# TencentARC/SEED-Story

Hardware: AMD Instinct MI355X
Metric: story-steps/sec (text + 1024x1024 image) (higher is better)
Workload: dtype bf16

## Files before the change

### seed-story_amd/csrc/ss_gemm.hip

```cpp
#include <stdio.h>

#include <map>
#include <mutex>

#include "ss_gemm_common.h"

namespace ss {

__device__ __attribute__((aligned(16))) unsigned int g_zero_page[64];

template <typename T, int BM, int BN, int WM, int WN, int KT, bool CONV, bool SPLIT = false>
__global__ __launch_bounds__(64 * WM * WN) void gemm_kernel(const GemmArgs g) {
    static_assert(!SPLIT || Tr<T>::kVec == 4, "SPLIT: fp32 operands");
    constexpr int V = Tr<T>::kVec;
    constexpr int NT = 64 * WM * WN;
    constexpr int PPR = 8 * KT;
    constexpr int BK = PPR * V;
    constexpr int LS = BK + V;
    constexpr int TM = BM / WM, TN = BN / WN;
    constexpr int FM = TM / 16, FN = TN / 16;
    constexpr int PA = (BM * PPR + NT - 1) / NT, PW = (BN * PPR + NT - 1) / NT;
    static_assert(TM % 16 == 0 && TN % 16 == 0, "wave tile must be MFMA-shaped");

    extern __shared__ __attribute__((aligned(16))) char smem_raw[];
// ... 231 lines not shown
    }
    if (g.conv_Cin > 0)
        hipLaunchKernelGGL((gemm_kernel<T, BM, BN, WM, WN, KT, true>), grid, dim3(64 * WM * WN), lds, s, g);
    else
        hipLaunchKernelGGL((gemm_kernel<T, BM, BN, WM, WN, KT, false>), grid, dim3(64 * WM * WN), lds, s, g);
    SS_LAUNCH_CHECK("gemm");
    return SS_OK;
}

template <typename T, int BM, int BN, int WM, int WN, int NS, bool CONV>
__global__ __launch_bounds__(64 * WM * WN) void gemm_glds_kernel(const GemmArgs g) {
    constexpr int V = 8;
    constexpr int NW = WM * WN;
    constexpr int BK = 64;
    constexpr int TM = BM / WM, TN = BN / WN;
    constexpr int FM = TM / 16, FN = TN / 16;
    constexpr int IA = BM / 8 / NW, IW = BN / 8 / NW;
    static_assert(BM % (8 * NW) == 0 && BN % (8 * NW) == 0, "tile rows must split evenly over the waves");
    extern __shared__ __attribute__((aligned(16))) char smem_raw[];
    constexpr int TILE_BYTES = (BM + BN) * 128;

    const int tid = threadIdx.x, lane = tid & 63;
    const int wid = __builtin_amdgcn_readfirstlane(tid >> 6);
    const int wm = wid / WN, wn = wid % WN;
    const int l15 = lane & 15, grp = lane >> 4;
    int mt_, nt_;
    xcd_tile(g.swz, (g.M + BM - 1) / BM, (g.N + BN - 1) / BN, mt_, nt_);
    const int m_blk = mt_ * BM, n_blk = nt_ * BN;
    const T* __restrict__ A = (const T*)g.A;
    const T* __restrict__ W = (const T*)g.W;
    const int K = g.K, M = g.M, N = g.N;
    const int ntiles = (K + BK - 1) / BK;
    const T* zero = reinterpret_cast<const T*>(g_zero_page);
    const uint32_t lds0 = __builtin_amdgcn_readfirstlane((uint32_t)(size_t)(lds_void_t*)smem_raw);

    const int srow = lane >> 3;
    const int schunk = (lane & 7) ^ srow;
    int cb[IA], cy[IA], cx[IA];
    if constexpr (CONV) {
#pragma unroll
        for (int i = 0; i < IA; ++i) {
            const int m = m_blk + (wid * IA + i) * 8 + srow;
            const int hw = g.conv_Ho * g.conv_Wo;
            cb[i] = m / hw;
            const int rem = m - cb[i] * hw;
            cy[i] = rem / g.conv_Wo;
            cx[i] = rem - cy[i] * g.conv_Wo;
        }
    }
    auto issue_tile = [&](int t, int buf) {
        const int k = t * BK + schunk * V;
        const uint32_t base = lds0 + (uint32_t)(buf * TILE_BYTES);
#pragma unroll
        for (int i = 0; i < IA; ++i) {
            const int r8 = (wid * IA + i) * 8;
            const int m = m_blk + r8 + srow;
            const T* src = zero;
            if constexpr (CONV) {
                int tap, ci;
                if ((g.conv_Cin & 63) == 0) {
                    const int k0 = t * BK;
                    tap = k0 / g.conv_Cin;
                    ci = k0 - tap * g.conv_Cin + schunk * V;
                } else {
                    tap = k / g.conv_Cin;
                    ci = k - tap * g.conv_Cin;
                }
                const int dy = tap / 3 - 1, dx = tap - (tap / 3) * 3 - 1;
                int iy = cy[i] * g.conv_stride + dy, ix = cx[i] * g.conv_stride + dx;
                const int Hin = g.conv_up ? 2 * g.conv_H : g.conv_H, Win = g.conv_up ? 2 * g.conv_W : g.conv_W;
                const bool ok = m < M && k < K && iy >= 0 && iy < Hin && ix >= 0 && ix < Win;
                if (g.conv_up) { iy >>= 1; ix >>= 1; }
                if (ok) src = A + (((int64_t)cb[i] * g.conv_H + iy) * g.conv_W + ix) * g.conv_Cin + ci;
            } else {
                if (m < M && k < K) src = A + (int64_t)m * g.lda + k;
            }
            dma16(src, __builtin_amdgcn_readfirstlane(base + (uint32_t)(r8 * 128)));
        }
#pragma unroll
        for (int i = 0; i < IW; ++i) {
            const int r8 = (wid * IW + i) * 8;
            const int n = n_blk + r8 + srow;
            const T* src = (n < N && k < K) ? W + (int64_t)n * g.ldw + k : zero;
            dma16(src, __builtin_amdgcn_readfirstlane(base + (uint32_t)((BM + r8) * 128)));
        }
    };

    f32x4_t acc[FN][FM];
#pragma unroll
    for (int i = 0; i < FN; ++i)
#pragma unroll
        for (int j = 0; j < FM; ++j) acc[i][j] = f32x4_t{0.f, 0.f, 0.f, 0.f};

    constexpr int IPT = IA + IW;
#pragma unroll
    for (int st = 0; st < NS - 1; ++st)
        if (st < ntiles) issue_tile(st, st);
    int buf = 0;
    for (int t = 0; t < ntiles; ++t) {
        if (t + NS - 2 < ntiles) wait_vmcnt<(NS - 2) * IPT>();
        else wait_vmcnt<0>();
        __syncthreads();
        if (t + NS - 1 < ntiles) {
            int nb = buf + NS - 1;
            if (nb >= NS) nb -= NS;
            issue_tile(t + NS - 1, nb);
        }
        const char* abuf = smem_raw + buf * TILE_BYTES;
        if (++buf == NS) buf = 0;
        const char* wbuf = abuf + BM * 128;
#pragma unroll
        for (int ks = 0; ks < 2; ++ks) {
            uint4 fw[FN], fa[FM];
#pragma unroll
            for (int i = 0; i < FN; ++i) {
                const int r = wn * TN + i * 16 + l15;
                fw[i] = *reinterpret_cast<const uint4*>(wbuf + r * 128 + (((ks * 4 + grp) ^ (r & 7)) << 4));
            }
#pragma unroll
            for (int j = 0; j < FM; ++j) {
                const int r = wm * TM + j * 16 + l15;
                fa[j] = *reinterpret_cast<const uint4*>(abuf + r * 128 + (((ks * 4 + grp) ^ (r & 7)) << 4));
            }
#pragma unroll
            for (int i = 0; i < FN; ++i)
#pragma unroll
                for (int j = 0; j < FM; ++j) acc[i][j] = Mma<T>::run(fw[i], fa[j], acc[i][j]);
        }
    }

    gemm_epilogue<T, FM, FN>(g, acc, m_blk + wm * TM, n_blk + wn * TN, l15, grp);
}

template <typename T, int BM, int BN, int WM, int WN, int NS>
static int gemm_glds_launch_cfg(const GemmArgs& g, hipStream_t s) {
    if constexpr (Tr<T>::kVec == 8) {
        const size_t lds = (size_t)NS * (BM + BN) * 128;
        dim3 grid((unsigned)cdiv(g.N, BN), (unsigned)cdiv(g.M, BM));
        if (g.conv_Cin > 0)
            hipLaunchKernelGGL((gemm_glds_kernel<T, BM, BN, WM, WN, NS, true>), grid, dim3(64 * WM * WN), lds, s, g);
        else
            hipLaunchKernelGGL((gemm_glds_kernel<T, BM, BN, WM, WN, NS, false>), grid, dim3(64 * WM * WN), lds, s, g);
        SS_LAUNCH_CHECK("gemm_glds");
        return SS_OK;
    } else {
        return gemm_launch_cfg<T, 128, 128, 2, 2>(g, s);
    }
}

template <> int gemm_sp_dispatch<float>(int, const GemmArgs&, hipStream_t) { return 1; }
template <> int gemm_sp_dispatch_conv<float>(int, const GemmArgs&, hipStream_t) { return 1; }
template <> int gemm_pp_dispatch<float>(int, const GemmArgs&, hipStream_t) { return 1; }
template <> int gemm_pp_dispatch_conv<float>(int, const GemmArgs&, hipStream_t) { return 1; }
template <> int gemm_w4_dispatch<float>(int, const GemmArgs&, hipStream_t) { return 1; }
template <> int gemm_w4_dispatch_conv<float>(int, const GemmArgs&, hipStream_t) { return 1; }

template <typename T>
static int gemm_dispatch_cfg(int cfg, const GemmArgs& g, hipStream_t s) {
    if (cfg >= 90 && cfg < 100 && Tr<T>::kVec == 8) {
        const int rc = gemm_w4_run<T>(cfg, g, s);
        if (rc <= 0) return rc;
        cfg = g.conv_Cin > 0 ? 69 : 60;
    }
    if (cfg >= 50 && cfg < 60 && Tr<T>::kVec == 8) {
        const int rc = gemm_pp_run<T>(cfg, g, s);
        if (rc <= 0) return rc;
        cfg = g.conv_Cin > 0 ? 69 : 60;
    }
    if (cfg >= 20 && Tr<T>::kVec == 8) {
        const int rc = gemm_sp_run<T>(cfg, g, s);
        if (rc <= 0) return rc;
        const GemmTile t = sp_tile(cfg);
        cfg = t.BM == 64 ? 10 : (t.BM == 128 && t.BN == 64) ? 15 : 8;
    }
    switch (cfg) {
        case 1:
            if constexpr (Tr<T>::kVec == 4) {
                if (knob(K_gemm_f32_split)) {
                    const int st = knob(K_gemm_f32_split_tile);
                    if (st == 1 || (st == 0 && g.conv_Cin == 0 && g.M >= 2048 && g.N >= 8192)) return gemm_launch_cfg<T, 256, 128, 4, 2>(g, s);
                    if (st == 2) return gemm_launch_cfg<T, 128, 256, 2, 4>(g, s);
                }
            }
            return gemm_launch_cfg<T, 128, 128, 2, 2>(g, s);
        case 2: return gemm_launch_cfg<T, 64, 64, 2, 2>(g, s);
        case 8: return gemm_glds_launch_cfg<T, 128, 128, 2, 2, 2>(g, s);
        case 10: return gemm_glds_launch_cfg<T, 64, 64, 2, 2, 2>(g, s);
        case 15: return gemm_glds_launch_cfg<T, 128, 64, 2, 2, 2>(g, s);
        default:
            if (cfg >= 20) return gemm_launch_cfg<T, 128, 128, 2, 2>(g, s);
            return gemm_launch_cfg<T, 128, 32, 4, 1>(g, s);
    }
}

struct TuneKey {
    int32_t v[8];
    bool operator<(const TuneKey& o) const {
        for (int i = 0; i < 8; ++i) if (v[i] != o.v[i]) return v[i] < o.v[i];
        return false;
    }
};
static std::mutex g_tune_mutex;
static std::map<TuneKey, int>& tune_cache() {
    static std::map<TuneKey, int> m;
    return m;
}
static TuneKey make_key(int dtype, const GemmArgs& g) {
    const bool conv = g.conv_Cin > 0;
    const int Mk = conv ? g.M : (g.M + 127) / 128 * 128;
    return TuneKey{{dtype, Mk, g.N, g.K, g.conv_Cin, conv ? g.conv_stride * 2 + g.conv_up : 0, conv ? g.conv_H : 0,
                    conv ? g.conv_W : 0}};
}

static int pick_cfg(const GemmArgs& g, bool f32) {
    const int force = knob(K_gemm_cfg);
    if (force) return force;
    const int64_t M = g.M, N = g.N;
    if (M <= 128) return 3;
    if (f32) return 1;
    const bool sp_ok = (g.K % 64 == 0) && (g.conv_Cin == 0 || g.conv_Cin % 64 == 0);
    const int64_t t256 = (int64_t)cdiv(M, 256), t128 = (int64_t)cdiv(M, 128);
    if (sp_ok) {
        if (N % 160 == 0 && N < 2560) {
            if (t256 * (N / 160) >= 200) return 62;
            if (t128 * (N / 160) >= 200) return 61;
            return 67;
        }
        if (t256 * cdiv(N, 256) >= 200) return g.conv_Cin > 0 ? 69 : 60;
        if (N % 160 == 0 && t128 * (N / 160) >= 200) return 61;
        if (t128 * cdiv(N, 128) >= 256) return 65;
        return t128 * cdiv(N, 64) >= 256 ? 68 : 70;
    }
    return t128 * cdiv(N, 128) >= 256 ? 8 : 10;
}

template <typename T>
static int lookup_cfg(GemmArgs& g) {
    const int fallback = pick_cfg(g, Tr<T>::kVec != 8);
    if (Tr<T>::kVec != 8 || g.M <= 128 || knob(K_gemm_cfg) || !knob(K_gemm_table)) return fallback;
    const TuneKey key = make_key(Tr<T>::kDtype, g);
    std::lock_guard<std::mutex> lk(g_tune_mutex);
    auto it = tune_cache().find(key);
    if (it == tune_cache().end()) return fallback;
    g.swz = it->second / 100;
    return it->second % 100;
}

__global__ void tune_fill_kernel(uint16_t* p, size_t n, uint32_t seed, int is_bf16, float scale) {
    for (size_t i = (size_t)blockIdx.x * blockDim.x + threadIdx.x; i < n; i += (size_t)gridDim.x * blockDim.x) {
        uint32_t x = (uint32_t)i * 2654435761u + seed;
        x ^= x >> 15; x *= 2246822519u; x ^= x >> 13; x *= 3266489917u; x ^= x >> 16;
        const float f = ((float)(x >> 8) * (1.0f / 8388608.0f) - 1.0f) * scale;
        p[i] = is_bf16 ? (uint16_t)f32_to_bf16_bits(f) : (uint16_t)f32_to_f16_bits(f);
    }
}

static size_t tune_rot_bytes(size_t w_bytes) {
    const size_t wb = (w_bytes + 255) / 256 * 256;
    size_t n = ((size_t)352 << 20) / wb;
    if (n > 128) n = 128;
    if (n < 2) n = 2;
    return n * wb;
}

static const int kTuneCands[] = {8, 15, 10, 22, 54, 55, 56, 57, 58, 60, 61, 62, 63, 64, 65, 66, 67, 68, 69, 70, 71, 72};

template <typename T>
static int tune_shape(GemmArgs g, void* ws, size_t ws_bytes, size_t a_elems, hipStream_t s, float* best_us) {
    if constexpr (Tr<T>::kVec != 8) {
        return SS_OK;
    } else {
        const size_t e = sizeof(T);
        auto up = [](size_t b) { return (b + 255) / 256 * 256; };
        const size_t a_b = up(a_elems * e), w_b = up((size_t)g.N * g.K * e), c_b = up((size_t)g.M * g.N * e);
        SS_REQUIRE(ws && ws_bytes >= a_b + 2 * w_b + c_b, "tune: workspace too small (%zu bytes)", ws_bytes);
        int nW = (int)((ws_bytes - a_b - c_b) / w_b);
        if (nW > 128) nW = 128;
        char* p = (char*)ws;
        g.A = p; g.C = p + a_b;
        char* w0 = p + a_b + c_b;
        g.epi &= SS_EPI_GEGLU_PAIR | SS_EPI_GELU;
        if (g.epi & SS_EPI_GEGLU_PAIR) g.ldc = g.N / 2;
        hipLaunchKernelGGL(tune_fill_kernel, dim3(2048), dim3(256), 0, s, (uint16_t*)g.A, a_elems, 0x1234u,
                           Tr<T>::kDtype == SS_BF16, 1.0f);
        hipLaunchKernelGGL(tune_fill_kernel, dim3(2048), dim3(256), 0, s, (uint16_t*)w0, (size_t)nW * (w_b / e), 0x9876u,
                           Tr<T>::kDtype == SS_BF16, 0.05f);
        SS_LAUNCH_CHECK("tune_fill");
        hipEvent_t e0, e1;
        SS_HIP(hipEventCreate(&e0));
        SS_HIP(hipEventCreate(&e1));
        const int swzs[3] = {0, 4, 8};
        int best = -1, best_swz = 0;
        float best_ms = 1e30f;
        const bool log = knob(K_gemm_autotune_log) != 0;
        const int R = nW + nW / 2 > 12 ? nW + nW / 2 : 12;
        for (int c : kTuneCands) {
            for (int z : swzs) {
                g.swz = z;
                g.W = w0;
                if (c >= 50 && c < 60) {
                    const int rc = gemm_pp_run<T>(c, g, s);
                    if (rc != SS_OK) break;
                }
                if (gemm_dispatch_cfg<T>(c, g, s) != SS_OK) continue;
                g.W = w0 + w_b; gemm_dispatch_cfg<T>(c, g, s);
                hipEventRecord(e0, s);
// ... 496 lines not shown
```

### seed-story_amd/csrc/ss_gemm_common.h

```cpp
#pragma once
#include <type_traits>
#include <utility>

#include "ss_common.h"

namespace ss {

typedef __attribute__((ext_vector_type(4))) uint32_t u32x4_t;
typedef __attribute__((ext_vector_type(8))) uint32_t u32x8_t;
template <int NV> struct Frag { uint4 v[NV]; };
template <typename T> struct OutT { using type = T; };
template <> struct OutT<fp8_t> { using type = bf16_t; };
template <typename T> struct Mma;
template <> struct Mma<bf16_t> {
    static constexpr int kK = 32;
    static constexpr int kEB = 2;
    static constexpr int kNV = 1;
    static __device__ __forceinline__ f32x4_t run(const uint4& a, const uint4& b, f32x4_t c) {
        return __builtin_amdgcn_mfma_f32_16x16x32_bf16(__builtin_bit_cast(bf16x8_t, a),
                                                       __builtin_bit_cast(bf16x8_t, b), c, 0, 0, 0);
    }
    static __device__ __forceinline__ void run_inplace(const uint4& a, const uint4& b, f32x4_t& c) {
        asm volatile("v_mfma_f32_16x16x32_bf16 %0, %1, %2, %0"
                     : "+v"(c)
// ... 532 lines not shown
#pragma unroll
            for (int r = 0; r < 4; ++r) t[r] = acc[i][c][r] + bv[i][r];
            if constexpr (EV == 2) {
#pragma unroll
                for (int r = 0; r < 4; ++r) t[r] = gelu_for<T>(Tr<T>::rnd(t[r]));
            }
            if constexpr (EV == 3) {
                float rv[8];
                asm volatile("" : "+v"(rvp[i].x), "+v"(rvp[i].y));
                unpack<T>(make_uint4(rvp[i].x, rvp[i].y, 0u, 0u), rv);
#pragma unroll
                for (int r = 0; r < 4; ++r) t[r] = Tr<T>::rnd(t[r]) + rv[r];
            }
            if constexpr (GEGLU) {
                float v0, v1, v2, v3;
                unpack2<T>(pack2<T>(t[0], t[1]), v0, v1);
                unpack2<T>(pack2<T>(t[2], t[3]), v2, v3);
                const float o0 = v0 * Tr<T>::rnd(gelu_for<T>(v1)), o1 = v2 * Tr<T>::rnd(gelu_for<T>(v3));
                *reinterpret_cast<uint32_t*>(wrow + i * 16) = pack2<T>(o0, o1);
            } else {
                *reinterpret_cast<uint2*>(wrow + i * 32) = make_uint2(pack2<T>(t[0], t[1]), pack2<T>(t[2], t[3]));
            }
        }
    };
    uint4 u[NP];
    auto readback = [&]() {
#pragma unroll
        for (int k = 0; k < NP; ++k) u[k] = *reinterpret_cast<const uint4*>(stg + loff[k]);
    };

    constexpr int RD = 2;
    uint4 rr[FM][NP];
    auto row_ok = [&](int c, int k) { return pv[k] && (WHOLE || m_base + c * 16 + prow[k] < M); };
    auto load_res = [&](int c) {
        const gmem_char_t* Rc = uniform_gptr(Rb + c * rstep);
#pragma unroll
        for (int k = 0; k < NP; ++k) {
            if constexpr (WHOLE) rr[c][k] = gmem_ld16(Rc + roff[k]);
            else rr[c][k] = row_ok(c, k) ? gmem_ld16(Rc + roff[k]) : make_uint4(0u, 0u, 0u, 0u);
        }
    };
    load_rv(0);
    if (has_res) {
#pragma unroll
        for (int c = 0; c < RD && c < FM; ++c) load_res(c);
    }
    __builtin_amdgcn_sched_barrier(0);
    stage(0);
    __builtin_amdgcn_sched_barrier(0);
    readback();
#pragma unroll
    for (int c = 0; c < FM; ++c) {
        if (has_res && c + RD < FM) load_res(c + RD);
        __builtin_amdgcn_sched_barrier(0);
        if (c + 1 < FM) stage(c + 1);
        __builtin_amdgcn_sched_barrier(0);
        gmem_char_t* Cc = uniform_gptr(Cb + c * cstep);
#pragma unroll
        for (int k = 0; k < NP; ++k) {
            uint4 o = u[k];
            if (has_res) {
                float a[8], b[8];
                unpack<T>(o, a);
                unpack<T>(rr[c][k], b);
#pragma unroll
                for (int e = 0; e < 8; ++e) a[e] += b[e];
                o = pack<T>(a);
            }
            if (row_ok(c, k)) gmem_st16(Cc + goff[k], o);
        }
        __builtin_amdgcn_sched_barrier(0);
        if (c + 1 < FM) readback();
    }
}

#define SS_SP_TILES(X) \
    X(20, 128, 128, 2, 2, 1, 2,  0, 0) \
    X(21, 128,  64, 2, 2, 1, 2,  0, 0) \
    X(22,  64,  64, 2, 2, 1, 2,  0, 0) \
    X(23, 256, 128, 4, 2, 1, 2,  0, 0) \
    X(24, 256, 256, 2, 4, 2, 2,  0, 0)    \
    X(26, 128, 160, 2, 2, 1, 2,  0, 0)    \
    X(28, 128, 320, 2, 4, 1, 2,  0, 0)    \
    X(29,  64, 160, 2, 2, 1, 2,  0, 0)    \
    X(30, 256, 160, 4, 2, 1, 2,  0, 0)    \
    X(31, 256, 160, 4, 2, 1, 3,  0, 0)    \
    X(32, 256, 160, 4, 2, 1, 3,  1, 0)    \
    X(33, 256, 160, 4, 2, 1, 3,  3, 0)    \
    X(34, 256, 256, 2, 4, 2, 2,  1, 0)    \
    X(35, 256, 256, 2, 4, 2, 2,  2, 0)    \
    X(36, 256, 256, 2, 4, 2, 2,  3, 0)    \
    X(37, 128, 160, 2, 2, 1, 2,  1, 0)    \
    X(38, 256, 160, 4, 2, 1, 2,  2, 0)    \
    X(39, 128, 320, 2, 4, 1, 2,  2, 0)    \
    X(40, 256, 256, 2, 4, 2, 2,  6, 0)    \
    X(41, 128, 160, 2, 2, 1, 2,  4, 0)    \
    X(42, 256, 160, 4, 2, 1, 3,  4, 0)    \
    X(43, 256, 160, 4, 2, 1, 2,  6, 0)    \
    X(44, 128, 320, 2, 4, 1, 2,  4, 0)    \
    X(45, 256, 128, 4, 2, 1, 2,  4, 0)    \
    X(46, 128, 128, 2, 2, 1, 2,  4, 0)    \
    X(60, 256, 256, 2, 4, 2, 2, 11, 1)    \
    X(61, 128, 160, 2, 2, 1, 2,  8, 3)    \
    X(62, 256, 160, 4, 2, 1, 3, 12, 3)    \
    X(63, 128, 320, 2, 4, 1, 2,  8, 3)    \
    X(64, 256, 160, 4, 2, 1, 2, 10, 3)    \
    X(65, 128, 128, 2, 2, 1, 2,  8, 3)    \
    X(66, 256, 128, 4, 2, 1, 2,  8, 1)    \
    X(67,  64, 160, 2, 2, 1, 2,  8, 3)    \
    X(68, 128,  64, 2, 2, 1, 2,  8, 1)    \
    X(69, 256, 256, 2, 4, 2, 2,  8, 1)    \
    X(70,  64,  64, 2, 2, 1, 2,  8, 1)    \
    X(71, 256, 160, 4, 2, 1, 2,  8, 3)    \
    X(72, 128, 320, 2, 4, 1, 2, 10, 3)
#define SS_SP_SPLITK_TILES(X) \
    X(300, 128, 128, 2, 2, 1, 2, 64, 0) \
    X(301, 128,  64, 2, 2, 1, 2, 64, 0)
#define SS_SP_FP8_TILES(X) \
    X(80, 128, 128, 2, 2, 2, 2, 8, 0)     \
    X(81, 128, 160, 2, 2, 2, 2, 8, 0)     \
    X(82, 256, 160, 4, 2, 2, 2, 8, 0)     \
    X(85,  64, 160, 2, 2, 1, 2, 8, 0)     \
    X(86,  64,  64, 2, 2, 1, 2, 8, 0) \
    X(88, 128, 160, 2, 2, 2, 2, 0, 0)
#define SS_W4_FP8_TILES(X) \
    X(95, 256, 256, 2, 2, 16, 0, 2, 0)    \
    X(96, 256, 256, 2, 2, 16, 0, 0, 0)

struct GemmTile { int id, BM, BN, WM, WN, NH, NS, FLAGS, variants; };
#define SS_TILE_ROW(id, BM, BN, WM, WN, NH, NS, FLAGS, VAR) {id, BM, BN, WM, WN, NH, NS, FLAGS, VAR},
constexpr GemmTile kSpTiles[] = {SS_SP_TILES(SS_TILE_ROW)};
constexpr GemmTile kFp8Tiles[] = {SS_SP_FP8_TILES(SS_TILE_ROW) SS_W4_FP8_TILES(SS_TILE_ROW)};
template <int N> constexpr GemmTile find_tile(const GemmTile (&t)[N], int id) {
    for (int i = 0; i < N; ++i) if (t[i].id == id) return t[i];
    return GemmTile{};
}
constexpr GemmTile sp_tile(int id) { return find_tile(kSpTiles, id); }
constexpr GemmTile fp8_tile(int id) { return find_tile(kFp8Tiles, id); }

template <int N> constexpr bool tiles_well_formed(const GemmTile (&t)[N]) {
    for (int i = 0; i < N; ++i) {
        for (int j = 0; j < i; ++j) if (t[j].id == t[i].id) return false;
        if (t[i].id < 1 || t[i].id >= 100 || (t[i].variants && !(t[i].FLAGS & 8))) return false;
    }
    return true;
}
static_assert(tiles_well_formed(kSpTiles) && tiles_well_formed(kFp8Tiles),
              "tile lists: duplicate id, base id outside 1 .. 99, or a variant on a tile without the staged epilogue");

template <typename T> int gemm_sp_dispatch(int cfg, const GemmArgs& g, hipStream_t s);
template <typename T> int gemm_sp_dispatch_conv(int cfg, const GemmArgs& g, hipStream_t s);
template <typename T> int gemm_pp_dispatch(int cfg, const GemmArgs& g, hipStream_t s);
template <typename T> int gemm_pp_dispatch_conv(int cfg, const GemmArgs& g, hipStream_t s);
template <typename T> int gemm_w4_dispatch(int cfg, const GemmArgs& g, hipStream_t s);
template <typename T> int gemm_w4_dispatch_conv(int cfg, const GemmArgs& g, hipStream_t s);
int gemm_sp_dispatch_fp8(int cfg, const GemmArgs& g, hipStream_t s);
int gemm_w4_dispatch_fp8(int cfg, const GemmArgs& g, hipStream_t s);
template <typename T> static int gemm_sp_run(int cfg, const GemmArgs& g, hipStream_t s) {
    return g.conv_Cin > 0 ? gemm_sp_dispatch_conv<T>(cfg, g, s) : gemm_sp_dispatch<T>(cfg, g, s);
}
template <typename T> static int gemm_pp_run(int cfg, const GemmArgs& g, hipStream_t s) {
    return g.conv_Cin > 0 ? gemm_pp_dispatch_conv<T>(cfg, g, s) : gemm_pp_dispatch<T>(cfg, g, s);
}
template <typename T> static int gemm_w4_run(int cfg, const GemmArgs& g, hipStream_t s) {
    return g.conv_Cin > 0 ? gemm_w4_dispatch_conv<T>(cfg, g, s) : gemm_w4_dispatch<T>(cfg, g, s);
}

static inline int num_cus() {
    static int n = 0;
    if (!n) {
        int dev = 0;
        hipDeviceProp_t p;
        if (hipGetDevice(&dev) == hipSuccess && hipGetDeviceProperties(&p, dev) == hipSuccess) n = p.multiProcessorCount;
        if (n <= 0) n = 256;
    }
    return n;
}
template <auto KERN> static int launch_tiles(const char* name, const GemmArgs& g, int total, int cap, int threads, size_t lds, hipStream_t s) {
    const int grid = cap > 0 && total > cap ? cap : total;
    if (lds > 64 * 1024) SS_DYN_LDS(KERN, lds);
    hipLaunchKernelGGL(KERN, dim3((unsigned)grid, (unsigned)g.ksplit), dim3(threads), lds, s, g, total);
    SS_LAUNCH_CHECK(name);
    return SS_OK;
}

}
```

### seed-story_amd/csrc/ss_gemm_pp.inc

```

namespace ss {

template <int BN, int FLAGS>
struct PpLds {
    static constexpr int FN = BN / 64, FN0 = (FN + 1) / 2, FN1 = FN / 2, TN = FN * 16;
    static constexpr int HA = 128 * 128, HB0 = 4 * FN0 * 16 * 128, HB1 = 4 * FN1 * 16 * 128;
    static constexpr int BUF = 2 * HA + HB0 + HB1;
    static constexpr int STG_CR = 16, STG_WAVE = STG_CR * (TN * 2 + 16);
    static constexpr bool STG_IN_RING = 2 * BUF + 8 * STG_WAVE > 163840;
    static constexpr int BYTES = 2 * BUF + ((FLAGS & 8) != 0 && !STG_IN_RING ? 8 * STG_WAVE : 0);
};

static __device__ __attribute__((aligned(4096))) unsigned int g_pp_zero_page[1024];

__device__ __forceinline__ void dma16v(const char* gsrc, uint32_t lds_base) {
    asm volatile(
        "s_mov_b32 m0, %1\n\t"
        "s_nop 0\n\t"
        "global_load_lds_dwordx4 %0, off"
        :
        : "v"(gsrc), "s"(lds_base)
        : "memory");
}

__device__ __forceinline__ void dma16s_at(uint32_t voff, const void* sbase, uint32_t lds_wave, int off) {
    asm volatile(
        "s_add_u32 m0, %2, %3\n\t"
        "s_nop 0\n\t"
        "global_load_lds_dwordx4 %0, %1"
        :
        : "v"(voff), "s"(sbase), "s"(lds_wave), "i"(off)
        : "memory", "scc");
}
__device__ __forceinline__ void dma16v_at(const char* gsrc, uint32_t lds_wave, int off) {
    asm volatile(
        "s_add_u32 m0, %1, %2\n\t"
        "s_nop 0\n\t"
        "global_load_lds_dwordx4 %0, off"
        :
        : "v"(gsrc), "s"(lds_wave), "i"(off)
        : "memory", "scc");
}

__device__ __forceinline__ uint32_t sel_lanes(uint32_t a, uint32_t b, uint64_t mask) {
    uint32_t r;
    asm("v_cndmask_b32 %0, %1, %2, %3" : "=v"(r) : "v"(a), "v"(b), "s"(mask));
    return r;
}
__device__ __forceinline__ uint64_t uniform_u64(uint64_t v) {
    const uint32_t lo = __builtin_amdgcn_readfirstlane((uint32_t)v), hi = __builtin_amdgcn_readfirstlane((uint32_t)(v >> 32));
    return ((uint64_t)hi << 32) | lo;
}

template <typename T, int BN, int FLAGS, bool CONV>
__global__ __launch_bounds__(512) void gemm_pp_kernel(const GemmArgs g, const int total_tiles) {
    using Lds = PpLds<BN, FLAGS>;
    constexpr int BM = 256, FN = Lds::FN, FN0 = Lds::FN0, FN1 = Lds::FN1, TM = 128, TN = Lds::TN, FM = 8;
    static_assert(BN == 256 || BN == 320, "tile widths");
    constexpr bool EXACT = BN == 320 || CONV;
    constexpr bool PRIO = (FLAGS & 1) != 0, PERSIST = (FLAGS & 2) != 0, TWO = (FLAGS & 4) != 0, STAGED = (FLAGS & 8) != 0, RSTAT = (FLAGS & 32) != 0;
    constexpr int EM = ((FLAGS & 16) != 0) ? 2 : 0;
    constexpr int HA = Lds::HA, HB0 = Lds::HB0, HB1 = Lds::HB1, BUF = Lds::BUF;
    constexpr int OFF_A0 = 0, OFF_A1 = HA, OFF_B0 = 2 * HA, OFF_B1 = 2 * HA + HB0;
    constexpr int NP0 = FN0, NP1 = FN1;
    constexpr int FLY = NP0 + 2 + NP1;
    constexpr int STG_CR = Lds::STG_CR, STG_WAVE = Lds::STG_WAVE;
    constexpr bool STG_IN_RING = Lds::STG_IN_RING;
    static_assert(!(PERSIST && STG_IN_RING), "persistent tiles prefetch under the epilogue: the strips need their own LDS");
    static_assert(Mma<T>::kEB == 2, "16-bit operands");
    using TO = T;
    extern __shared__ __attribute__((aligned(16))) char smem_raw[];

    const int tid = threadIdx.x, lane = tid & 63;
    const int wid = __builtin_amdgcn_readfirstlane(tid >> 6);
    const int wm = wid >> 2, wn = wid & 3;
    const int l15 = lane & 15, grp = lane >> 4;
    const int M = g.M, N = g.N;
    const int MT = (M + BM - 1) / BM, NT = (N + BN - 1) / BN;
    const int ntiles = g.K / 64;
    const int tpt = CONV ? g.conv_Cin / 64 : 1;
    const uint32_t tpt_inv = CONV ? (65536u + (uint32_t)tpt - 1u) / (uint32_t)tpt : 0u;
    const int lw = CONV ? __builtin_ctz((unsigned)g.conv_W) : 0;
    const uint32_t lds0 = __builtin_amdgcn_readfirstlane((uint32_t)(size_t)(lds_void_t*)smem_raw);

    const int srow = lane >> 3;
    const int schunk = (lane & 7) ^ srow;
    auto b_col = [&](int h, int i) {
        const int RH = (h ? FN1 : FN0) * 16;
        const int r8 = (wid + 8 * i) * 8;
        return (r8 / RH) * TN + (h ? FN0 * 16 : 0) + r8 % RH + srow;
    };
    int m_blk = 0, n_blk = 0;
    uint32_t voffA[EXACT ? 1 : 2][EXACT ? 1 : 2], voffW[EXACT ? 1 : 2][EXACT ? 1 : 3];
    const char* sbaseA = nullptr;
    const char* sbaseW = nullptr;
    uint32_t cpoff[CONV ? 2 : 1][CONV ? 2 : 1];
    uint64_t cpad = 0, crow = 0;
    auto setup_tile = [&](int vid) {
        int mt_, nt_;
        xcd_tile_id(g.swz, MT, NT, vid, mt_, nt_);
        m_blk = mt_ * BM; n_blk = nt_ * BN;
        if constexpr (CONV) {
            voffA[0][0] = (uint32_t)(srow * g.conv_Cin * 2 + schunk * 16);
            voffW[0][0] = (uint32_t)((int64_t)srow * g.ldw * 2 + schunk * 16);
            uint64_t pad = 0, row = 0;
#pragma unroll
            for (int h = 0; h < 2; ++h) {
#pragma unroll
                for (int i = 0; i < 2; ++i) {
                    const int m0 = m_blk + i * 128 + h * 64 + wid * 8;
                    const int y0 = (m0 >> lw) & (g.conv_H - 1), x0 = m0 & (g.conv_W - 1);
                    const uint64_t r9 = (y0 == 0 ? 0x000000111ull : 0ull) | (y0 == g.conv_H - 1 ? 0x111000000ull : 0ull);
                    const uint64_t p9 = r9 | (x0 == 0 ? 0x001001001ull : 0ull) | (x0 + 8 == g.conv_W ? 0x100100100ull : 0ull);
                    row |= r9 << (h * 2 + i);
                    pad |= p9 << (h * 2 + i);
                    cpoff[h][i] = __builtin_amdgcn_readfirstlane((uint32_t)(m0 * g.conv_Cin * 2));
                }
            }
            cpad = uniform_u64(pad); crow = uniform_u64(row);
        } else if constexpr (EXACT) {
            voffA[0][0] = (uint32_t)((int64_t)srow * g.lda * 2 + schunk * 16);
            voffW[0][0] = (uint32_t)((int64_t)srow * g.ldw * 2 + schunk * 16);
        } else {
#pragma unroll
            for (int h = 0; h < 2; ++h) {
#pragma unroll
                for (int i = 0; i < 2; ++i) {
                    int m = m_blk + i * 128 + h * 64 + wid * 8 + srow;
                    m = m < M ? m : M - 1;
                    voffA[h][i] = (uint32_t)((int64_t)(m - m_blk) * g.lda * 2 + schunk * 16);
                }
#pragma unroll
                for (int i = 0; i < (h ? NP1 : NP0); ++i) {
                    int n = n_blk + b_col(h, i);
                    n = n < N ? n : N - 1;
                    voffW[h][i] = (uint32_t)((int64_t)(n - n_blk) * g.ldw * 2 + schunk * 16);
                }
            }
        }
        sbaseA = uniform_ptr((const char*)g.A + (CONV ? (int64_t)0 : (int64_t)m_blk * g.lda * 2));
        sbaseW = uniform_ptr((const char*)g.W + (int64_t)n_blk * g.ldw * 2);
    };
    struct Cur { const char* src; int c, tap; uint32_t bits; };
    auto cur_set_tap = [&](Cur& k) {
        const int t3 = (k.tap * 11) >> 5;
        const int dy = t3 - 1, dx = k.tap - 3 * t3 - 1;
        k.src = (const char*)g.A + ((int64_t)(dy * g.conv_W + dx) * g.conv_Cin + k.c * 64) * 2;
        k.bits = ((uint32_t)(cpad >> (k.tap * 4)) & 15u) | (((uint32_t)(crow >> (k.tap * 4)) & 15u) << 4) | (dx < 0 ? 256u : 0u);
    };
    auto cur_make = [&](int t) {
        Cur k;
        k.tap = (int)(((uint32_t)t * tpt_inv) >> 16);
        k.c = t - k.tap * tpt;
        cur_set_tap(k);
        return k;
    };
    auto cur_next = [&](Cur& k) {
        k.c += 1; k.src += 128;
        if (k.c == tpt) { k.c = 0; k.tap += 1; cur_set_tap(k); }
    };
    const uint32_t ldsw = lds0 + (uint32_t)(wid * 1024);
    const uint64_t zaddr = (uint64_t)(size_t)g_pp_zero_page;
    const uint32_t zlo = (uint32_t)zaddr | (uint32_t)((tid & 255) << 4);
    uint32_t zhi = (uint32_t)(zaddr >> 32);
    if constexpr (CONV && BN == 256) asm volatile("" : "+v"(zhi));
    auto stage_conv = [&](const Cur& k, int b, int h) {
        const uint32_t keep = m0_save();
#pragma unroll
        for (int i = 0; i < 2; ++i) {
            const int p = h * 2 + i;
            const char* ps = k.src + cpoff[CONV ? h : 0][CONV ? i : 0];
            const int d = b * BUF + (h ? OFF_A1 : OFF_A0) + i * 8192;
            if (__builtin_expect(((k.bits >> p) & 1u) == 0, 1)) {
                dma16s_at(voffA[0][0], ps, ldsw, d);
            } else {
                const uint64_t zm = ((k.bits >> (4 + p)) & 1u) ? ~0ull : ((k.bits & 256u) ? 0xFFull : 0xFFull << 56);
                const uint64_t a = (uint64_t)(size_t)ps + voffA[0][0];
                const uint32_t lo = sel_lanes((uint32_t)a, zlo, zm), hi = sel_lanes((uint32_t)(a >> 32), zhi, zm);
                dma16v_at((const char*)(size_t)(((uint64_t)hi << 32) | lo), ldsw, d);
            }
        }
        m0_restore(keep);
    };
    auto stage = [&](int t, int b, int which) {
        const uint32_t keep = m0_save();
        const int h = which & 1;
        if (which < 2) {
            const uint32_t dst = lds0 + (uint32_t)(b * BUF + (h ? OFF_A1 : OFF_A0) + wid * 1024);
            const char* src = sbaseA + (int64_t)t * 128;
#pragma unroll
            for (int i = 0; i < 2; ++i) {
                if constexpr (CONV) {
                } else if constexpr (EXACT)
                    dma16s(voffA[0][0], uniform_ptr(src + (int64_t)(i * 128 + h * 64 + wid * 8) * g.lda * 2), __builtin_amdgcn_readfirstlane(dst + i * 8192u));
                else
                    dma16s(voffA[h][i], src, __builtin_amdgcn_readfirstlane(dst + i * 8192u));
            }
        } else {
            const uint32_t dst = lds0 + (uint32_t)(b * BUF + (h ? OFF_B1 : OFF_B0) + wid * 1024);
            const char* src = sbaseW + (int64_t)t * 128;
#pragma unroll
            for (int i = 0; i < (h ? NP1 : NP0); ++i) {
                if constexpr (CONV)
                    dma16s_at(voffW[0][0], src + (uint32_t)__builtin_amdgcn_readfirstlane((b_col(h, i) - srow) * g.ldw * 2), ldsw,
                              b * BUF + (h ? OFF_B1 : OFF_B0) + i * 8192);
                else if constexpr (EXACT)
                    dma16s(voffW[0][0], uniform_ptr(src + (int64_t)(b_col(h, i) - srow) * g.ldw * 2), __builtin_amdgcn_readfirstlane(dst + i * 8192u));
                else
                    dma16s(voffW[h][i], src, __builtin_amdgcn_readfirstlane(dst + i * 8192u));
            }
        }
        m0_restore(keep);
    };
    auto prologue = [&]() {
        if constexpr (CONV) {
            const Cur k0 = cur_make(0);
            stage(0, 0, 2); stage_conv(k0, 0, 0); stage(0, 0, 3); stage_conv(k0, 0, 1);
            if (ntiles > 1) { stage_conv(cur_make(1), 1, 0); stage(1, 1, 2); if constexpr (!TWO) stage(1, 1, 3); }
        } else {
            stage(0, 0, 2); stage(0, 0, 0); stage(0, 0, 3); stage(0, 0, 1);
            if (ntiles > 1) { stage(1, 1, 0); stage(1, 1, 2); if constexpr (!TWO) stage(1, 1, 3); }
        }
    };

    const uint32_t fsw = (uint32_t)((grp ^ (l15 & 7)) << 4);
    const uint32_t fa0 = (uint32_t)((wm * 64 + l15) * 128) + fsw, fa1 = fa0 ^ 64u;
    const uint32_t fw00 = (uint32_t)((wn * FN0 * 16 + l15) * 128) + fsw, fw01 = fw00 ^ 64u;
    const uint32_t fw10 = (uint32_t)((wn * FN1 * 16 + l15) * 128) + fsw, fw11 = fw10 ^ 64u;
    uint4 fa[4][2], fw0[FN0][2], fw1[FN1][2];
    auto read_a = [&](const char* half) {
#pragma unroll
        for (int j = 0; j < 4; ++j) {
            fa[j][0] = *reinterpret_cast<const uint4*>(half + fa0 + j * 2048);
            fa[j][1] = *reinterpret_cast<const uint4*>(half + fa1 + j * 2048);
        }
    };
    auto read_w0 = [&](const char* half) {
#pragma unroll
        for (int i = 0; i < FN0; ++i) {
            fw0[i][0] = *reinterpret_cast<const uint4*>(half + fw00 + i * 2048);
            fw0[i][1] = *reinterpret_cast<const uint4*>(half + fw01 + i * 2048);
        }
    };
    auto read_w1 = [&](const char* half) {
#pragma unroll
        for (int i = 0; i < FN1; ++i) {
            fw1[i][0] = *reinterpret_cast<const uint4*>(half + fw10 + i * 2048);
            fw1[i][1] = *reinterpret_cast<const uint4*>(half + fw11 + i * 2048);
        }
    };
    f32x4_t acc[FN][FM];
    auto mma = [&](int h, auto hp_tag) {
        constexpr int hp = decltype(hp_tag)::value;
        if constexpr (PRIO) __builtin_amdgcn_s_setprio(1);
#pragma unroll
        for (int ks = 0; ks < 2; ++ks)
#pragma unroll
            for (int i = 0; i < (hp ? FN1 : FN0); ++i)
#pragma unroll
                for (int j = 0; j < 4; ++j) {
                    if constexpr (hp == 0) Mma<T>::run_inplace(fw0[i][ks], fa[j][ks], acc[i][h * 4 + j]);
                    else Mma<T>::run_inplace(fw1[i][ks], fa[j][ks], acc[FN0 + i][h * 4 + j]);
                }
        if constexpr (PRIO) __builtin_amdgcn_s_setprio(0);
    };
    constexpr std::integral_constant<int, 0> H0{};
    constexpr std::integral_constant<int, 1> H1{};
    auto bar = [&]() { __builtin_amdgcn_s_barrier(); };
    auto pin = [&]() { __builtin_amdgcn_sched_barrier(0); };

    int vid = blockIdx.x;
    setup_tile(vid);
    prologue();
    bool first = true;

    while (true) {
        const int m_cur = m_blk, n_cur = n_blk;
        const int vnext = vid + (int)gridDim.x;
        const bool has_next = PERSIST && vnext < total_tiles;
#pragma unroll
        for (int i = 0; i < FN; ++i)
#pragma unroll
            for (int j = 0; j < FM; ++j) acc[i][j] = f32x4_t{0.f, 0.f, 0.f, 0.f};
        if (first && ntiles > 1) wait_vmcnt<(TWO ? 2 + NP0 : FLY)>(); else wait_vmcnt<0>();
        first = false;
        bar();
#pragma unroll
        for (int i = 0; i < FN; ++i)
#pragma unroll
            for (int j = 0; j < FM; ++j) asm volatile("" : "+v"(acc[i][j]));
        asm volatile("s_nop 7" ::: "memory");
        if (wm == 1) bar();
        Cur P1 = cur_make(CONV ? 1 : 0), P2 = cur_make(CONV ? 2 : 0);

        auto tile = [&](int t, auto btag) {
            constexpr int b = decltype(btag)::value;
            const char* L = smem_raw + b * BUF;
            const bool s1 = t + 1 < ntiles, s2 = t + 2 < ntiles;
            read_w0(L + OFF_B0);
            pin();
            read_a(L + OFF_A0);
            pin();
            if (s1) { if constexpr (CONV) stage_conv(P1, b ^ 1, 1); else stage(t + 1, b ^ 1, 1); }
            asm volatile("s_waitcnt lgkmcnt(8)" ::: "memory");
            bar();
            asm volatile("s_waitcnt lgkmcnt(0)" ::: "memory");
            pin();
            mma(0, H0);
            pin();
            bar();
            read_w1(L + OFF_B1);
            pin();
            if (s2) stage(t + 2, b, 2);
            bar();
            asm volatile("s_waitcnt lgkmcnt(0)" ::: "memory");
            pin();
            mma(0, H1);
            pin();
            bar();
            read_a(L + OFF_A1);
            pin();
            if (s2) { if constexpr (CONV) stage_conv(P2, b, 0); else stage(t + 2, b, 0); }
            bar();
            asm volatile("s_waitcnt lgkmcnt(0)" ::: "memory");
            pin();
            mma(1, H1);
            pin();
            bar();
            if (s2) { stage(t + 2, b, 3); wait_vmcnt<FLY>(); } else { wait_vmcnt<0>(); }
            bar();
            pin();
            mma(1, H0);
            pin();
            bar();
            if constexpr (CONV) { P1 = P2; cur_next(P2); }
        };
        auto tile2 = [&](int t, auto btag) {
            constexpr int b = decltype(btag)::value;
            const char* L = smem_raw + b * BUF;
            const bool s1 = t + 1 < ntiles, s2 = t + 2 < ntiles;
            read_w0(L + OFF_B0);
            read_w1(L + OFF_B1);
            read_a(L + OFF_A0);
            pin();
            if (s1) {
                stage(t + 1, b ^ 1, 3);
                if constexpr (CONV) stage_conv(P1, b ^ 1, 1); else stage(t + 1, b ^ 1, 1);
                wait_vmcnt<4 + NP0 + NP1>();
            } else {
                wait_vmcnt<0>();
            }
            asm volatile("s_waitcnt lgkmcnt(0)" ::: "memory");
            bar();
            pin();
            mma(0, H0);
            mma(0, H1);
            pin();
            bar();
            read_a(L + OFF_A1);
            pin();
            if (s2) {
                if constexpr (CONV) stage_conv(P2, b, 0); else stage(t + 2, b, 0);
                stage(t + 2, b, 2);
                wait_vmcnt<4 + NP0>();
            } else if (s1) {
                wait_vmcnt<2>();
            } else {
                wait_vmcnt<0>();
            }
            asm volatile("s_waitcnt lgkmcnt(0)" ::: "memory");
            bar();
            pin();
            mma(1, H1);
            mma(1, H0);
            pin();
            bar();
            if constexpr (CONV) { P1 = P2; cur_next(P2); }
        };
        int t = 0;
        for (; t + 1 < ntiles; t += 2) {
            if constexpr (TWO) { tile2(t, std::integral_constant<int, 0>{}); tile2(t + 1, std::integral_constant<int, 1>{}); }
            else { tile(t, std::integral_constant<int, 0>{}); tile(t + 1, std::integral_constant<int, 1>{}); }
        }
        if (t < ntiles) { if constexpr (TWO) tile2(t, std::integral_constant<int, 0>{}); else tile(t, std::integral_constant<int, 0>{}); }
        if (wm == 0) bar();

        if (has_next) {
            setup_tile(vnext);
            prologue();
        }
        asm volatile("s_nop 15\n\ts_nop 15" ::: "memory");
#pragma unroll
        for (int i = 0; i < FN; ++i)
#pragma unroll
            for (int j = 0; j < FM; ++j) asm volatile("" : "+v"(acc[i][j]));

        bool staged = false;
        if constexpr (STAGED) {
            constexpr size_t A16 = 15;
            staged = (n_cur + wn * TN + TN <= N) && (((size_t)g.C | (size_t)g.residual | (size_t)g.bias | (size_t)g.rowvec) & A16) == 0 &&
                     ((g.ldc | g.ldr | g.rowvec_ld) & 7) == 0 && (EM == 0 || ((size_t)g.scale_w & A16) == 0);
            if (staged) {
                char* strip = smem_raw + (STG_IN_RING ? 0 : 2 * BUF) + wid * STG_WAVE;
                const int mb = m_cur + wm * TM, nb = n_cur + wn * TN;
                const bool o_gelu = (g.epi & SS_EPI_GELU) != 0, o_geglu = (g.epi & SS_EPI_GEGLU_PAIR) != 0;
                const bool o_rv = g.rowvec != nullptr || (!CONV && (g.epi & SS_EPI_INTERNAL_GENERIC) != 0);
                if constexpr (EM == 0 && !RSTAT) {
                    const bool o_res = (g.epi & SS_EPI_RESIDUAL) != 0;
                    if (!o_gelu && !o_geglu && !o_rv && !o_res) gemm_epilogue_staged_pipe<TO, FM, FN, 1, false, EXACT>(g, acc, mb, nb, lane, strip);
                    else if (!o_gelu && !o_geglu && !o_rv) gemm_epilogue_staged_pipe<TO, FM, FN, 1, true, EXACT>(g, acc, mb, nb, lane, strip);
                    else if (CONV && !o_gelu && !o_geglu && !o_res && (g.rows_per_batch & 15) == 0) gemm_epilogue_staged_pipe<TO, FM, FN, 3, false, EXACT>(g, acc, mb, nb, lane, strip);
                    else if (!CONV && o_geglu && !o_gelu && !o_rv && !o_res) gemm_epilogue_staged_pipe<TO, FM, FN, 4, false, EXACT>(g, acc, mb, nb, lane, strip);
                    else if (!CONV && o_gelu && !o_geglu && !o_rv && !o_res) gemm_epilogue_staged_pipe<TO, FM, FN, 2, false, EXACT>(g, acc, mb, nb, lane, strip);
                    else gemm_epilogue_staged<TO, FM, FN, STG_CR, EM, RSTAT, 0>(g, acc, mb, nb, lane, strip);
                } else {
                if (!o_gelu && !o_geglu && !o_rv) gemm_epilogue_staged<TO, FM, FN, STG_CR, EM, RSTAT, 1>(g, acc, mb, nb, lane, strip);
                else if constexpr (CONV) gemm_epilogue_staged<TO, FM, FN, STG_CR, EM, RSTAT, 3>(g, acc, mb, nb, lane, strip);
                else if (o_geglu && !o_gelu && !o_rv) gemm_epilogue_staged<TO, FM, FN, STG_CR, EM, RSTAT, 4>(g, acc, mb, nb, lane, strip);
                else if (o_gelu && !o_geglu && !o_rv) gemm_epilogue_staged<TO, FM, FN, STG_CR, EM, RSTAT, 2>(g, acc, mb, nb, lane, strip);
                else gemm_epilogue_staged<TO, FM, FN, STG_CR, EM, RSTAT, 0>(g, acc, mb, nb, lane, strip);
                }
            }
        }
        if (!staged) gemm_epilogue<TO, FM, FN, EM, RSTAT>(g, acc, m_cur + wm * TM, n_cur + wn * TN, l15, grp);
        if (!has_next) break;
        vid = vnext;
        asm volatile("" : "+s"(vid));
        setup_tile(vid);
    }
}

template <typename T, int BN, int FLAGS>
static int pp_launch(const GemmArgs& g, hipStream_t s) {
    constexpr bool CONV = SS_PP_CONV != 0;
    const bool conv = g.conv_Cin > 0;
    if (conv != CONV || g.ksplit > 1) return 1;
    bool ok = (g.K % 64 == 0) && g.K >= 64 && (int64_t)BN * g.ldw * 2 < (1ll << 31);
    if (conv) {
        ok = ok && g.conv_stride == 1 && !g.conv_up && g.conv_Cin % 64 == 0 && g.conv_Cin <= 4096 && g.conv_W >= 8 &&
             (g.conv_W & (g.conv_W - 1)) == 0 && (g.conv_H & (g.conv_H - 1)) == 0 && g.M % 256 == 0 && g.N % BN == 0 &&
             (int64_t)g.M * g.conv_Cin * 2 < (1ll << 31);
    } else {
        ok = ok && (int64_t)256 * g.lda * 2 < (1ll << 31);
        if (BN == 320 && (g.M % 256 != 0 || g.N % 320 != 0)) ok = false;
    }
    if (!ok) return 1;
    if ((g.rowstat_out || g.rowpart) && !(FLAGS & 32)) return 1;
    return launch_tiles<gemm_pp_kernel<T, BN, FLAGS, CONV>>("gemm_pp", g, cdiv(g.M, 256) * cdiv(g.N, BN), (FLAGS & 2) ? num_cus() : 0, 512,
                                                            PpLds<BN, FLAGS>::BYTES, s);
}

#if SS_PP_CONV
template <typename T> int gemm_pp_dispatch_conv(int cfg, const GemmArgs& g, hipStream_t s) {
#else
template <typename T> int gemm_pp_dispatch(int cfg, const GemmArgs& g, hipStream_t s) {
#endif
    switch (cfg) {
        case 54: return pp_launch<T, 256, 8>(g, s);
        case 55: return pp_launch<T, 256, 10>(g, s);
        case 56: return pp_launch<T, 320, 8>(g, s);
        case 57: return pp_launch<T, 256, 12>(g, s);
#if !SS_PP_CONV
        case 58: return pp_launch<T, 320, 12>(g, s);
#endif
        default: return 1;
    }
}
#if SS_PP_CONV
template int gemm_pp_dispatch_conv<SS_PP_T>(int, const GemmArgs&, hipStream_t);
#else
template int gemm_pp_dispatch<SS_PP_T>(int, const GemmArgs&, hipStream_t);
#endif

}
```

Baseline: 2.441.

## Add fused nearest-upsample implicit-GEMM conv path to ping-pong GEMM kernel

Adds an UP variant of the ping-pong implicit-GEMM conv kernel that reads the pre-upsample input directly. It computes source offsets, odd-row shifts and padding masks for the 2x nearest-upsampled geometry. Upsample convs (e.g. in the VAE decoder) previously could not use the pp kernel and fell back to slower paths, or needed a materialized upsampled tensor. The change adds per-tap offset computation and more registers, and whether it runs depends on the autotuned cfg selecting 54/56/57 for upsampling convs.

```diff
diff --git a/seed-story_amd/csrc/ss_conv_up.h b/seed-story_amd/csrc/ss_conv_up.h
--- /dev/null
+++ b/seed-story_amd/csrc/ss_conv_up.h
@@ -0,0 +1,46 @@
+#pragma once
+#include <stdint.h>
+
+#if defined(__HIPCC__) || defined(__CUDACC__)
+#define SS_UP_HD __host__ __device__ __forceinline__
+#else
+#define SS_UP_HD inline
+#endif
+
+namespace ss {
+
+struct UpPiece {
+    uint32_t off;
+    uint32_t odd;
+    uint64_t row9;
+    uint64_t pad9;
+};
+
+SS_UP_HD UpPiece up_piece(int m0, int lwo, int Ho, int Wo, int Cin) {
+    const int ox0 = m0 & (Wo - 1), r = m0 >> lwo;
+    const int oy = r & (Ho - 1);
+    const int sp = (((r - oy) >> 1) + (oy >> 1)) * (Wo >> 1) + (ox0 >> 1);
+    UpPiece p;
+    p.off = (uint32_t)sp * (uint32_t)Cin * 2u;
+    p.odd = (uint32_t)(oy & 1);
+    p.row9 = (oy == 0 ? 0x000000111ull : 0ull) | (oy == Ho - 1 ? 0x111000000ull : 0ull);
+    p.pad9 = p.row9 | (ox0 == 0 ? 0x001001001ull : 0ull) | (ox0 + 8 == Wo ? 0x100100100ull : 0ull);
+    return p;
+}
+
+SS_UP_HD uint32_t up_shift_bits(uint32_t odd, int piece) { return (odd ? 0x100u : 0x001u) << piece; }
+
+SS_UP_HD uint32_t up_piece_off(uint32_t off, uint32_t shift, int piece, int dyi, uint32_t row_bytes) {
+    const uint32_t d = dyi == 0 ? 0u - row_bytes : row_bytes;
+    return off + (((shift >> (dyi * 4 + piece)) & 1u) ? d : 0u);
+}
+
+SS_UP_HD int64_t up_tap_off(int dx, int c, int Cin) { return ((int64_t)(dx < 0 ? -Cin : 0) + (int64_t)c * 64) * 2; }
+
+SS_UP_HD uint32_t up_lane_off(int i, int chunk, int Cin, bool odd) {
+    return (uint32_t)(((i + (odd ? 1 : 0)) >> 1) * Cin * 2 + chunk * 16);
+}
+
+SS_UP_HD uint64_t up_pad_lanes(bool whole_row, bool dx_neg) { return whole_row ? ~0ull : (dx_neg ? 0xFFull : 0xFFull << 56); }
+
+}
diff --git a/seed-story_amd/csrc/ss_gemm.hip b/seed-story_amd/csrc/ss_gemm.hip
--- a/seed-story_amd/csrc/ss_gemm.hip
+++ b/seed-story_amd/csrc/ss_gemm.hip
@@ -407,6 +407,7 @@
 template <> int gemm_sp_dispatch_conv<float>(int, const GemmArgs&, hipStream_t) { return 1; }
 template <> int gemm_pp_dispatch<float>(int, const GemmArgs&, hipStream_t) { return 1; }
 template <> int gemm_pp_dispatch_conv<float>(int, const GemmArgs&, hipStream_t) { return 1; }
+template <> int gemm_pp_dispatch_convup<float>(int, const GemmArgs&, hipStream_t) { return 1; }
 template <> int gemm_w4_dispatch<float>(int, const GemmArgs&, hipStream_t) { return 1; }
 template <> int gemm_w4_dispatch_conv<float>(int, const GemmArgs&, hipStream_t) { return 1; }
 
diff --git a/seed-story_amd/csrc/ss_gemm_common.h b/seed-story_amd/csrc/ss_gemm_common.h
--- a/seed-story_amd/csrc/ss_gemm_common.h
+++ b/seed-story_amd/csrc/ss_gemm_common.h
@@ -708,6 +708,7 @@
 template <typename T> int gemm_sp_dispatch_conv(int cfg, const GemmArgs& g, hipStream_t s);
 template <typename T> int gemm_pp_dispatch(int cfg, const GemmArgs& g, hipStream_t s);
 template <typename T> int gemm_pp_dispatch_conv(int cfg, const GemmArgs& g, hipStream_t s);
+template <typename T> int gemm_pp_dispatch_convup(int cfg, const GemmArgs& g, hipStream_t s);
 template <typename T> int gemm_w4_dispatch(int cfg, const GemmArgs& g, hipStream_t s);
 template <typename T> int gemm_w4_dispatch_conv(int cfg, const GemmArgs& g, hipStream_t s);
 int gemm_sp_dispatch_fp8(int cfg, const GemmArgs& g, hipStream_t s);
@@ -716,7 +717,8 @@
     return g.conv_Cin > 0 ? gemm_sp_dispatch_conv<T>(cfg, g, s) : gemm_sp_dispatch<T>(cfg, g, s);
 }
 template <typename T> static int gemm_pp_run(int cfg, const GemmArgs& g, hipStream_t s) {
-    return g.conv_Cin > 0 ? gemm_pp_dispatch_conv<T>(cfg, g, s) : gemm_pp_dispatch<T>(cfg, g, s);
+    if (g.conv_Cin > 0) return g.conv_up ? gemm_pp_dispatch_convup<T>(cfg, g, s) : gemm_pp_dispatch_conv<T>(cfg, g, s);
+    return gemm_pp_dispatch<T>(cfg, g, s);
 }
 template <typename T> static int gemm_w4_run(int cfg, const GemmArgs& g, hipStream_t s) {
     return g.conv_Cin > 0 ? gemm_w4_dispatch_conv<T>(cfg, g, s) : gemm_w4_dispatch<T>(cfg, g, s);
diff --git a/seed-story_amd/csrc/ss_gemm_pp.inc b/seed-story_amd/csrc/ss_gemm_pp.inc
--- a/seed-story_amd/csrc/ss_gemm_pp.inc
+++ b/seed-story_amd/csrc/ss_gemm_pp.inc
@@ -1,3 +1,5 @@
+
+#include "ss_conv_up.h"
 
 namespace ss {
 
@@ -52,11 +54,12 @@
     return ((uint64_t)hi << 32) | lo;
 }
 
-template <typename T, int BN, int FLAGS, bool CONV>
+template <typename T, int BN, int FLAGS, bool CONV, bool UP = false>
 __global__ __launch_bounds__(512) void gemm_pp_kernel(const GemmArgs g, const int total_tiles) {
     using Lds = PpLds<BN, FLAGS>;
     constexpr int BM = 256, FN = Lds::FN, FN0 = Lds::FN0, FN1 = Lds::FN1, TM = 128, TN = Lds::TN, FM = 8;
     static_assert(BN == 256 || BN == 320, "tile widths");
+    static_assert(CONV || !UP, "upsampling is a conv input");
     constexpr bool EXACT = BN == 320 || CONV;
     constexpr bool PRIO = (FLAGS & 1) != 0, PERSIST = (FLAGS & 2) != 0, TWO = (FLAGS & 4) != 0, STAGED = (FLAGS & 8) != 0, RSTAT = (FLAGS & 32) != 0;
     constexpr int EM = ((FLAGS & 16) != 0) ? 2 : 0;
@@ -80,7 +83,8 @@
     const int ntiles = g.K / 64;
     const int tpt = CONV ? g.conv_Cin / 64 : 1;
     const uint32_t tpt_inv = CONV ? (65536u + (uint32_t)tpt - 1u) / (uint32_t)tpt : 0u;
-    const int lw = CONV ? __builtin_ctz((unsigned)g.conv_W) : 0;
+    const int cWo = UP ? 2 * g.conv_W : g.conv_W, cHo = UP ? 2 * g.conv_H : g.conv_H;
+    const int lw = CONV ? __builtin_ctz((unsigned)cWo) : 0;
     const uint32_t lds0 = __builtin_amdgcn_readfirstlane((uint32_t)(size_t)(lds_void_t*)smem_raw);
 
     const int srow = lane >> 3;
@@ -96,11 +100,31 @@
     const char* sbaseW = nullptr;
     uint32_t cpoff[CONV ? 2 : 1][CONV ? 2 : 1];
     uint64_t cpad = 0, crow = 0;
+    uint32_t cshift = 0, voffA_odd = 0;
     auto setup_tile = [&](int vid) {
         int mt_, nt_;
         xcd_tile_id(g.swz, MT, NT, vid, mt_, nt_);
         m_blk = mt_ * BM; n_blk = nt_ * BN;
-        if constexpr (CONV) {
+        if constexpr (UP) {
+            voffA[0][0] = up_lane_off(srow, schunk, g.conv_Cin, false);
+            voffA_odd = up_lane_off(srow, schunk, g.conv_Cin, true);
+            voffW[0][0] = (uint32_t)((int64_t)srow * g.ldw * 2 + schunk * 16);
+            uint64_t pad = 0, row = 0;
+            uint32_t shift = 0;
+#pragma unroll
+            for (int h = 0; h < 2; ++h) {
+#pragma unroll
+                for (int i = 0; i < 2; ++i) {
+                    const UpPiece q = up_piece(m_blk + i * 128 + h * 64 + wid * 8, lw, cHo, cWo, g.conv_Cin);
+                    row |= q.row9 << (h * 2 + i);
+                    pad |= q.pad9 << (h * 2 + i);
+                    shift |= up_shift_bits(q.odd, h * 2 + i);
+                    cpoff[h][i] = __builtin_amdgcn_readfirstlane(q.off);
+                }
+            }
+            cpad = uniform_u64(pad); crow = uniform_u64(row);
+            cshift = __builtin_amdgcn_readfirstlane(shift);
+        } else if constexpr (CONV) {
             voffA[0][0] = (uint32_t)(srow * g.conv_Cin * 2 + schunk * 16);
             voffW[0][0] = (uint32_t)((int64_t)srow * g.ldw * 2 + schunk * 16);
             uint64_t pad = 0, row = 0;
@@ -141,15 +165,23 @@
         sbaseA = uniform_ptr((const char*)g.A + (CONV ? (int64_t)0 : (int64_t)m_blk * g.lda * 2));
         sbaseW = uniform_ptr((const char*)g.W + (int64_t)n_blk * g.ldw * 2);
     };
-    struct Cur { const char* src; int c, tap; uint32_t bits; };
+    struct Cur { const char* src; int c, tap; uint32_t bits; uint32_t po[2][2]; };
     auto cur_set_tap = [&](Cur& k) {
         const int t3 = (k.tap * 11) >> 5;
         const int dy = t3 - 1, dx = k.tap - 3 * t3 - 1;
-        k.src = (const char*)g.A + ((int64_t)(dy * g.conv_W + dx) * g.conv_Cin + k.c * 64) * 2;
-        k.bits = ((uint32_t)(cpad >> (k.tap * 4)) & 15u) | (((uint32_t)(crow >> (k.tap * 4)) & 15u) << 4) | (dx < 0 ? 256u : 0u);
+        if constexpr (UP) {
+            k.src = (const char*)g.A + up_tap_off(dx, k.c, g.conv_Cin);
+            const uint32_t row_bytes = (uint32_t)(g.conv_W * g.conv_Cin * 2);
+#pragma unroll
+            for (int p = 0; p < 4; ++p) k.po[p >> 1][p & 1] = up_piece_off(cpoff[CONV ? p >> 1 : 0][CONV ? p & 1 : 0], cshift, p, t3, row_bytes);
+        } else {
+            k.src = (const char*)g.A + ((int64_t)(dy * g.conv_W + dx) * g.conv_Cin + k.c * 64) * 2;
+        }
+        k.bits = ((uint32_t)(cpad >> (k.tap * 4)) & 15u) | (((uint32_t)(crow >> (k.tap * 4)) & 15u) << 4) | (dx < 0 ? 256u : 0u) |
+                 (UP && dx != 0 ? 512u : 0u);
     };
     auto cur_make = [&](int t) {
-        Cur k;
+        Cur k{};
         k.tap = (int)(((uint32_t)t * tpt_inv) >> 16);
         k.c = t - k.tap * tpt;
         cur_set_tap(k);
@@ -166,16 +198,17 @@
     if constexpr (CONV && BN == 256) asm volatile("" : "+v"(zhi));
     auto stage_conv = [&](const Cur& k, int b, int h) {
         const uint32_t keep = m0_save();
+        const uint32_t vo = UP && (k.bits & 512u) ? voffA_odd : voffA[0][0];
 #pragma unroll
         for (int i = 0; i < 2; ++i) {
             const int p = h * 2 + i;
-            const char* ps = k.src + cpoff[CONV ? h : 0][CONV ? i : 0];
+            const char* ps = k.src + (UP ? k.po[h][i] : cpoff[CONV ? h : 0][CONV ? i : 0]);
             const int d = b * BUF + (h ? OFF_A1 : OFF_A0) + i * 8192;
             if (__builtin_expect(((k.bits >> p) & 1u) == 0, 1)) {
-                dma16s_at(voffA[0][0], ps, ldsw, d);
+                dma16s_at(vo, ps, ldsw, d);
             } else {
-                const uint64_t zm = ((k.bits >> (4 + p)) & 1u) ? ~0ull : ((k.bits & 256u) ? 0xFFull : 0xFFull << 56);
-                const uint64_t a = (uint64_t)(size_t)ps + voffA[0][0];
+                const uint64_t zm = up_pad_lanes(((k.bits >> (4 + p)) & 1u) != 0, (k.bits & 256u) != 0);
+                const uint64_t a = (uint64_t)(size_t)ps + vo;
                 const uint32_t lo = sel_lanes((uint32_t)a, zlo, zm), hi = sel_lanes((uint32_t)(a >> 32), zhi, zm);
                 dma16v_at((const char*)(size_t)(((uint64_t)hi << 32) | lo), ldsw, d);
             }
@@ -432,41 +465,48 @@
 
 template <typename T, int BN, int FLAGS>
 static int pp_launch(const GemmArgs& g, hipStream_t s) {
-    constexpr bool CONV = SS_PP_CONV != 0;
+    constexpr bool CONV = SS_PP_CONV != 0, UP = SS_PP_CONV == 2;
     const bool conv = g.conv_Cin > 0;
-    if (conv != CONV || g.ksplit > 1) return 1;
+    if (conv != CONV || (conv && (g.conv_up != 0) != UP) || g.ksplit > 1) return 1;
     bool ok = (g.K % 64 == 0) && g.K >= 64 && (int64_t)BN * g.ldw * 2 < (1ll << 31);
     if (conv) {
-        ok = ok && g.conv_stride == 1 && !g.conv_up && g.conv_Cin % 64 == 0 && g.conv_Cin <= 4096 && g.conv_W >= 8 &&
-             (g.conv_W & (g.conv_W - 1)) == 0 && (g.conv_H & (g.conv_H - 1)) == 0 && g.M % 256 == 0 && g.N % BN == 0 &&
-             (int64_t)g.M * g.conv_Cin * 2 < (1ll << 31);
+        const int Wo = g.conv_up ? 2 * g.conv_W : g.conv_W, Ho = g.conv_up ? 2 * g.conv_H : g.conv_H;
+        ok = ok && g.conv_stride == 1 && g.conv_Cin % 64 == 0 && g.conv_Cin <= 4096 && g.conv_W > 0 && g.conv_H > 0 && Wo >= 8 &&
+             (Wo & (Wo - 1)) == 0 && (Ho & (Ho - 1)) == 0 && g.M % 256 == 0 && g.N % BN == 0 &&
+             (int64_t)(g.conv_up ? g.M / 4 : g.M) * g.conv_Cin * 2 < (1ll << 31);
     } else {
         ok = ok && (int64_t)256 * g.lda * 2 < (1ll << 31);
         if (BN == 320 && (g.M % 256 != 0 || g.N % 320 != 0)) ok = false;
     }
     if (!ok) return 1;
     if ((g.rowstat_out || g.rowpart) && !(FLAGS & 32)) return 1;
-    return launch_tiles<gemm_pp_kernel<T, BN, FLAGS, CONV>>("gemm_pp", g, cdiv(g.M, 256) * cdiv(g.N, BN), (FLAGS & 2) ? num_cus() : 0, 512,
+    return launch_tiles<gemm_pp_kernel<T, BN, FLAGS, CONV, UP>>("gemm_pp", g, cdiv(g.M, 256) * cdiv(g.N, BN), (FLAGS & 2) ? num_cus() : 0, 512,
                                                             PpLds<BN, FLAGS>::BYTES, s);
 }
 
-#if SS_PP_CONV
+#if SS_PP_CONV == 2
+template <typename T> int gemm_pp_dispatch_convup(int cfg, const GemmArgs& g, hipStream_t s) {
+#elif SS_PP_CONV
 template <typename T> int gemm_pp_dispatch_conv(int cfg, const GemmArgs& g, hipStream_t s) {
 #else
 template <typename T> int gemm_pp_dispatch(int cfg, const GemmArgs& g, hipStream_t s) {
 #endif
     switch (cfg) {
         case 54: return pp_launch<T, 256, 8>(g, s);
+#if SS_PP_CONV != 2
         case 55: return pp_launch<T, 256, 10>(g, s);
+#endif
         case 56: return pp_launch<T, 320, 8>(g, s);
         case 57: return pp_launch<T, 256, 12>(g, s);
-#if !SS_PP_CONV
+#if SS_PP_CONV != 2
         case 58: return pp_launch<T, 320, 12>(g, s);
 #endif
         default: return 1;
     }
 }
-#if SS_PP_CONV
+#if SS_PP_CONV == 2
+template int gemm_pp_dispatch_convup<SS_PP_T>(int, const GemmArgs&, hipStream_t);
+#elif SS_PP_CONV
 template int gemm_pp_dispatch_conv<SS_PP_T>(int, const GemmArgs&, hipStream_t);
 #else
 template int gemm_pp_dispatch<SS_PP_T>(int, const GemmArgs&, hipStream_t);
diff --git a/seed-story_amd/csrc/ss_gemm_pp_bf16_convup.hip b/seed-story_amd/csrc/ss_gemm_pp_bf16_convup.hip
--- /dev/null
+++ b/seed-story_amd/csrc/ss_gemm_pp_bf16_convup.hip
@@ -0,0 +1,4 @@
+#include "ss_gemm_common.h"
+#define SS_PP_T ::ss::bf16_t
+#define SS_PP_CONV 2
+#include "ss_gemm_pp.inc"
diff --git a/seed-story_amd/csrc/ss_gemm_pp_f16_convup.hip b/seed-story_amd/csrc/ss_gemm_pp_f16_convup.hip
--- /dev/null
+++ b/seed-story_amd/csrc/ss_gemm_pp_f16_convup.hip
@@ -0,0 +1,4 @@
+#include "ss_gemm_common.h"
+#define SS_PP_T ::ss::f16_t
+#define SS_PP_CONV 2
+#include "ss_gemm_pp.inc"
```

Result: faster. 2.480, median of 6 (+1.6%).
